# qwerty35/swarm_simulator

Hardware: AMD Instinct MI355X
Metric: agent-trajectories/sec (RBP plan: SFC+RSFC+QP) (higher is better)
Workload: dtype f64

## Files before the change

swarm_simulator_amd/csrc/abi/session.hip:

```cpp
#include <cmath>
#include <cstdio>
#include <cstdlib>
#include <cstring>
#include <string>
#include <thread>
#include <vector>

#include "../kernels/jqp.h"
#include "../kernels/rbp_dev.h"

namespace {

thread_local std::string g_err;

int fail(int code, const std::string& msg) {
    g_err = msg;
    return code;
}

#define HIP_TRY(expr)                                                                                    \
    do {                                                                                                 \
        hipError_t e_ = (expr);                                                                          \
        if (e_ != hipSuccess)                                                                            \
            return fail(e_ == hipErrorNoDevice || e_ == hipErrorInvalidDevice ? RBP_ERR_NO_DEVICE : RBP_ERR_HIP, \
// ... 490 lines not shown
    HIP_TRY(hipMemsetAsync(d.status, 0, sizeof(int) * K, st));
    HIP_TRY(hipMemsetAsync(d.scalars, 0, sizeof(double) * K * SC_N, st));
    HIP_TRY(hipMemsetAsync(d.counters, 0, sizeof(unsigned long long) * K * CT_N, st));
    if (s->have_corridor_inputs) {
        HIP_TRY(hipMemcpyAsync(d.sfc_count, s->sfc_count0.data(), sizeof(int) * (size_t)K * N, hipMemcpyHostToDevice, st));
        HIP_TRY(hipMemcpyAsync(d.sfc_box, s->sfc_box0.data(), sizeof(double) * (size_t)K * N * MB * 6, hipMemcpyHostToDevice, st));
        HIP_TRY(hipMemcpyAsync(d.sfc_time, s->sfc_time0.data(), sizeof(double) * (size_t)K * N * MB, hipMemcpyHostToDevice, st));
        HIP_TRY(hipMemcpyAsync(d.rsfc_normal, s->rsfc_normal0.data(), sizeof(float) * (size_t)K * d.npair * M * 3, hipMemcpyHostToDevice, st));
        HIP_TRY(hipMemcpyAsync(d.rsfc_time, s->rsfc_time0.data(), sizeof(double) * (size_t)K * M, hipMemcpyHostToDevice, st));
    }
    return RBP_OK;
}

int rbp_session_set_agent_range(rbp_session* s, int32_t agent_begin, int32_t agent_end) {
    if (!s) return fail(RBP_ERR_BAD_ARGUMENT, "null session");
    if (int jrc = join_worker(s)) return jrc;
    if (agent_begin < 0 || agent_end < agent_begin || agent_end > s->d.N) return fail(RBP_ERR_BAD_ARGUMENT, "agent range outside [0, N]");
    s->d.agent_begin = agent_begin, s->d.agent_end = agent_end;
    return RBP_OK;
}

static int ensure_planner_workspace(rbp_session* s, hipStream_t st) {
    const DevSession& d = s->d;
    const int N = d.N, M = d.M, K = d.K;
    const rbp_solver_opts& o = s->opts;
    const bool joint_wide = !s->param.sequential && s->biter > 0 && N >= 2 && o.joint_wide_min_agents > 0 && N >= o.joint_wide_min_agents;
    if (!joint_wide) {
        if (M > QP_MAX_M) return fail(RBP_ERR_BAD_ARGUMENT, "more than " + std::to_string(QP_MAX_M) + " segments per mission are not supported by the QP kernel");
        if (s->biter > 0 && s->bs > planner_max_batch())
            return fail(RBP_ERR_BAD_ARGUMENT, "batch wider than " + std::to_string(planner_max_batch()) +
                                                  " agents (joint QP of a large mission) is not supported by the one-workgroup QP kernel "
                                                  "(rbp_solver_opts.joint_wide_min_agents selects the grid-wide solver)");
    }
    const size_t per = joint_wide ? joint_workspace_bytes(N, M) : std::max(planner_workspace_bytes_w2(N, M, s->bs), planner_workspace_bytes_w4(N, M, s->bs));
    s->joint_wide = joint_wide;
    if (s->qp_ws && s->ws_joint == joint_wide && s->qp_ws_per_mission == per) return RBP_OK;
    const size_t total = per * (size_t)K + 256;
    auto too_large = [&](hipError_t e) {
        return fail(RBP_ERR_HIP, "QP workspace: " + std::to_string(total) + " bytes (" + std::to_string(K) + " missions x " + std::to_string(per) +
                                     " bytes for " + (joint_wide ? "the grid-wide joint solver" : "the batch QP kernels") + ") could not be reserved: " +
                                     hipGetErrorString(e));
    };
    char* base = nullptr;
    if (s->ctx) {
        rbp_ctx* c = s->ctx;
        if (c->ws_cap < total) {
            HIP_TRY(hipStreamSynchronize(st));
            if (c->ws_base) (void)hipFree(c->ws_base);
            c->ws_base = nullptr, c->ws_cap = 0;
            const size_t want = total + total / 4;
            hipError_t e = hipMalloc((void**)&c->ws_base, want);
            if (e != hipSuccess) return too_large(e);
            c->ws_cap = want;
        }
        base = c->ws_base;
    } else {
        if (s->ws_own) {
            HIP_TRY(hipStreamSynchronize(st));
            (void)hipFree(s->ws_own);
            s->ws_own = nullptr;
        }
        hipError_t e = hipMalloc((void**)&s->ws_own, total);
        if (e != hipSuccess) return too_large(e);
        base = s->ws_own;
    }
    HIP_TRY(hipMemsetAsync(base, 0, total, st));
    s->qp_ws = base, s->qp_ws_per_mission = per, s->ws_joint = joint_wide;
    return RBP_OK;
}

size_t rbp_session_workspace_bytes(rbp_session* s) { return s && s->qp_ws ? s->qp_ws_per_mission : 0; }

int rbp_session_reserve_workspace(rbp_session* s, void* stream) {
    if (!s) return fail(RBP_ERR_BAD_ARGUMENT, "null session");
    if (int jrc = join_worker(s)) return jrc;
    HIP_TRY(hipSetDevice(s->device));
    return ensure_planner_workspace(s, (hipStream_t)stream);
}

int rbp_session_set_solver_opts(rbp_session* s, const rbp_solver_opts* o) {
    if (!s) return fail(RBP_ERR_BAD_ARGUMENT, "null session");
    if (int jrc = join_worker(s)) return jrc;
    int rc = check_solver_opts(o);
    if (rc) return rc;
    s->opts = *o;
    return RBP_OK;
}

static int run_impl(rbp_session* s, int stages, void* stream, bool async) {
    if (!s) return fail(RBP_ERR_BAD_ARGUMENT, "null session");
    if (int jrc = join_worker(s)) return jrc;
    hipStream_t st = (hipStream_t)stream;
    HIP_TRY(hipSetDevice(s->device));
    const rbp_solver_opts& o = s->opts;
    if (stages & RBP_STAGE_PLANNER) {
        int rc = ensure_planner_workspace(s, st);
        if (rc) return rc;
        if (s->shard.nranks == 2 && !s->joint_wide)
            return fail(RBP_ERR_BAD_ARGUMENT, "rbp_session_shard_joint: this plan does not run on the grid-wide joint solver (rbp_solver_opts.joint_wide_min_agents), there is no factorisation to share");
        if (s->shard.nranks == 2 && async)
// ... 508 lines not shown
```

swarm_simulator_amd/csrc/kernels/qp.hip:

```cpp
#include <algorithm>
#include <type_traits>
#include <vector>

#include "rbp_dev.h"

#pragma clang fp contract(fast)

#include "knot_lds.inc"
#include "common/ipm_rows.h"

#ifndef QP_THREADS
#define QP_THREADS 512
#endif
#define QP_MAX_ITERS 80
#ifndef QP_WARM_TAU
#define QP_WARM_TAU 1e-3
#endif
#ifndef QP_MU0
#define QP_MU0 3e-1
#endif
#ifndef QP_ROW_UNROLL
#define QP_ROW_UNROLL 2
#endif
#ifndef QP_ROW_PF
// ... 8 lines not shown
#ifndef QP_FAR_SLACK
#define QP_FAR_SLACK 0.7
#endif
#ifndef QP_SIGMA_POW
#define QP_SIGMA_POW 3
#endif
#ifndef QP_NBHD_GAMMA
#define QP_NBHD_GAMMA 1e-3
#endif
#ifndef QP_NBHD_BACKOFF
#define QP_NBHD_BACKOFF 0.8
#endif
#ifndef QP_STEP_FRAC
#define QP_STEP_FRAC 0.997
#endif
#ifndef QP_SFLOOR
#define QP_SFLOOR 1e-1
#endif
#ifndef QP_WAVES_PER_EU
#define QP_WAVES_PER_EU 2
#endif
#ifndef QP_CHAIN_PRIO
#define QP_CHAIN_PRIO 3
#endif
#ifndef QP_STAGE_BUFS
#define QP_STAGE_BUFS (QP_THREADS >= 512 ? 3 : 2)
#endif
#ifndef QP_STAGE_REGS
#define QP_STAGE_REGS (QP_THREADS >= 512 ? 0 : 2)
#endif
#ifndef QP_MID_FOLLOW
#define QP_MID_FOLLOW (QP_THREADS >= 512)
#endif
#ifndef QP_FWD_IN_FACTOR
#ifdef QP_TRACE
#define QP_FWD_IN_FACTOR 0
#else
#define QP_FWD_IN_FACTOR 1
#endif
#endif
#if QP_FWD_IN_FACTOR && KL_FUSED_UPDATE && KL_PANEL && KL_PANEL_MIN_NK <= 36
#define QP_FWD36 1
#else
#define QP_FWD36 0
#endif
#ifndef QP_EARLY_TRIES
#define QP_EARLY_TRIES 2
#endif
#ifndef QP_EARLY_TOL
#define QP_EARLY_TOL 1e-6
#endif
#include "lh_layout.h"
#define PL_NC 256
#define PL_PMAX 160
#define PL_PBIG 192
__host__ __device__ inline int polish_pmax(int nk) { return nk <= 36 ? 112 : PL_PMAX; }
__host__ __device__ inline size_t polish_s_doubles(int nj) { return std::max((size_t)PL_NC * PL_NC, ipm::k0g_doubles(nj)); }
__host__ __device__ inline size_t polish_ws_doubles(int nj, int nk) {
    return 18 * (size_t)nj + 2 + ipm::k0g_doubles(nj) + PL_NC * 14 + polish_s_doubles(nj) + 8 + lhp_size(PL_PBIG) + 4 * 6 * PL_PBIG + 3 * (size_t)nj * nk;
}
__host__ __device__ inline int polish_lds_doubles(int nk) {
    const int pm = polish_pmax(nk);
    return lhp_size(pm) + 3 * PL_NC + 3 * pm + (pm + 2 * PL_NC + 8) / 2 + 8;
}

namespace {
using namespace ipm;

#include "qp_base.inc"
#include "qp_polish_types.inc"
#include "qp_rows.inc"
#include "qp_newton.inc"
#include "qp_wave_factor.inc"
#include "qp_wave_solve.inc"
#include "qp_tiled.inc"
#include "qp_entries.inc"
#include "qp_polish.inc"
#include "qp_batch.inc"

__global__ __launch_bounds__(QP_THREADS, QP_WAVES_PER_EU) void qp_batch_kernel(DevSession S, double* ws_base, size_t ws_stride, int passes,
                                                               int biter, int nbmax, int lds_doubles) {
    const int mission = S.qp_order ? __builtin_amdgcn_readfirstlane(S.qp_order[blockIdx.x]) : (int)blockIdx.x;
    const long long t_start = wall_clock64();
    __shared__ DevSession S_lds;
    if (threadIdx.x == 0) S_lds = S;
// ... 84 lines not shown
```

swarm_simulator_amd/csrc/kernels/qp_base.inc:

```

#ifdef QP_PROFILE
#define PROF_DECL long long prof_t0 = wall_clock64(), prof_acc[12] = {0, 0, 0, 0, 0, 0, 0, 0, 0, 0, 0, 0}
#define PROF(i)                                \
    do {                                       \
        __syncthreads();                       \
        long long t_ = wall_clock64();         \
        prof_acc[i] += t_ - prof_t0;           \
        prof_t0 = t_;                          \
    } while (0)
#define PROF_FLUSH(scal)                                                         \
    do {                                                                         \
        if (threadIdx.x == 0)                                                    \
            for (int i_ = 0; i_ < 12; ++i_) scal[SC_PROF0 + i_] += (double)prof_acc[i_]; \
    } while (0)
#else
#define PROF_DECL
#define PROF(i)
#define PROF_FLUSH(scal)
#endif

struct QpDims {
    int N, M, oq;
    int nb, NF, npb;
    int nk, nj, ld;
// ... 44 lines not shown
}

__host__ __device__ inline size_t ws_doubles(int N, int M, int nbmax) {
    QpDims d = make_dims(N, M, 0, nbmax);
    size_t n = 7 * d.nslot_max + 12 * (size_t)nbmax * d.oq + (size_t)(d.npb ? d.npb : 1) * d.oq + 3 * (size_t)nbmax * 3 * d.oq +
               2 * (size_t)d.nj * d.nk + (size_t)d.nj * d.ldb * d.ldb + 2 * (size_t)d.nj * (d.nk < 36 ? d.nk : 36) * (d.nk < 36 ? d.nk : 36) +
               (size_t)(d.nj > 1 ? d.nj - 1 : 1) * d.ldb * d.ldb + 4 +
               2 * (size_t)nbmax * M * 3 + 3 * (size_t)(M + 1) * 9 + M + 64 + (ws_int_count(N, M, nbmax) + 1) / 2 + 2 +
                polish_ws_doubles(d.nj, d.nk);
    return n;
}

__device__ inline QpWs carve(double* base, const QpDims& d, int nbmax) {
    QpDims dm = make_dims(d.N, d.M, 0, nbmax);
    QpWs w;
    double* p = base;
    w.s = p, p += dm.nslot_max;
    w.z = p, p += dm.nslot_max;
    w.s2 = p, p += dm.nslot_max;
    w.z2 = p, p += dm.nslot_max;
    w.rh = p, p += dm.nslot_max;
    w.cc = p, p += dm.nslot_max;
    w.ds = p, p += dm.nslot_max;
    w.cpacc = p, p += 12 * (size_t)nbmax * d.oq;
    w.pwgt = p, p += (size_t)(dm.npb ? dm.npb : 1) * d.oq;
    w.dx = p, p += (size_t)nbmax * 3 * d.oq;
    w.dxa = p, p += (size_t)nbmax * 3 * d.oq;
    w.cvec = p, p += (size_t)nbmax * 3 * d.oq;
    w.rbase = p, p += (size_t)dm.nj * dm.nk;
    w.rhs = p, p += (size_t)dm.nj * dm.nk;
    p += (4 - ((p - base) & 3)) & 3;
    w.Td = p, p += (size_t)dm.nj * dm.ldb * dm.ldb;
    w.To = p, p += (size_t)(dm.nj > 1 ? dm.nj - 1 : 1) * dm.ldb * dm.ldb;
    w.Lf = p, p += 2 * (size_t)dm.nj * (dm.nk < 36 ? dm.nk : 36) * (dm.nk < 36 ? dm.nk : 36);
    w.boxlo = p, p += (size_t)nbmax * d.M * 3;
    w.boxhi = p, p += (size_t)nbmax * d.M * 3;
    w.Lk = p, p += (size_t)(d.M + 1) * 9;
    w.Dk = p, p += (size_t)(d.M + 1) * 9;
    w.Ek = p, p += (size_t)(d.M + 1) * 9;
    w.segsc = p, p += d.M;
    int* ip = (int*)p;
    w.flist = ip, ip += (size_t)nbmax * d.M * d.N;
    w.fnear = ip, ip += (size_t)nbmax * d.M;
    w.fcnt = ip, ip += (size_t)nbmax * d.M;
    w.fbase = ip, ip += (size_t)nbmax * d.M;
    w.fperm = ip, ip += (size_t)nbmax * d.M;
    w.frank = ip, ip += (size_t)nbmax * d.M;
    w.tile_base = ip, ip += dm.ntile + 1;
    w.wi_of = ip, ip += (size_t)nbmax * d.oq;
    w.nrm = (float*)ip;
    w.polish = p + (ws_int_count(d.N, d.M, nbmax) + 1) / 2 + 2;
    w.prof = nullptr;
    return w;
}

template <int CTRL>
__device__ __forceinline__ double dpp_f64(double v) {
    const int lo = __builtin_amdgcn_update_dpp(0, __double2loint(v), CTRL, 0xf, 0xf, false);
    const int hi = __builtin_amdgcn_update_dpp(0, __double2hiint(v), CTRL, 0xf, 0xf, false);
    return __hiloint2double(hi, lo);
}
__device__ __forceinline__ double red_op(double a, double b, int op) { return op == 0 ? a + b : (op == 1 ? fmax(a, b) : fmin(a, b)); }
__device__ __forceinline__ double rl(double v, int lane) {
    return __hiloint2double(__builtin_amdgcn_readlane(__double2hiint(v), lane), __builtin_amdgcn_readlane(__double2loint(v), lane));
}
__device__ __forceinline__ double wave_red(double v, int op ) {
    v = red_op(v, dpp_f64<0xB1>(v), op);
// ... 103 lines not shown
```

swarm_simulator_amd/csrc/kernels/qp_batch.inc:

```

#ifdef QP_TRACE
#ifndef QP_TRACE_BATCH
#define QP_TRACE_BATCH 0
#endif
#define TRC(slot, expr)                                                         \
    do {                                                                        \
        if (batch == QP_TRACE_BATCH && pass_index == 0 && iter < 100) {                       \
            const double v_ = (expr);                                           \
            if (tid == 0) trc[iter * 16 + (slot)] = v_;                         \
        }                                                                       \
    } while (0)
__device__ double trc_sum(const double* p, size_t n, double* red) {
    double a = 0;
    for (size_t i = threadIdx.x; i < n; i += QP_THREADS) a += fabs(p[i]);
    return block_reduce(a, 0, red);
}
#else
#define TRC(slot, expr)
#endif

__device__ __forceinline__ bool qp_setup_batch(const DevSession& S, RowCtx& c, double* ctrl, const double* T, int mission, int first, int nb,
                                               int* flag, double* lds, int& frozen_free_rows, double far_R, int& nfar) {
    const int tid = threadIdx.x, N = S.N;
    const QpDims& d = c.d;
// ... 326 lines not shown
        const bool early = early_tries < QP_EARLY_TRIES && pres < QP_EARLY_TOL && dres < QP_EARLY_TOL &&
                           mu < (early_tries == 0 ? QP_EARLY_TOL : 1e-2 * QP_EARLY_TOL);
        if (S.p.polish && (polish_first || early)) {
            if (!polish_first) early_tries++;
            const int acc = polish_entry(c, pw, lds, red, flag, polish_first ? 1 : 0);
            __syncthreads();
            PROF(0);
#ifdef QP_POLSTATS
            if (tid == 0 && !polish_first) scal[25] += (early_tries == 1), scal[26] += (early_tries == 1 && acc == 0), scal[27] += (early_tries == 2), scal[29] += (early_tries == 2 && acc == 0);
#endif
            if (acc == 0) {
                ok = true, polished = 1;
                break;
            }
        }
        if (d.nk > 36)
            assemble_blocks(c, lds);
        else if (ASM_HELPERS == 0 && !QP_FOLLOW_ASM)
            assemble_blocks_lds(asm_args(c), d.nj, lds);
#if QP_FWD36
        if (d.nk == 36) rhs_from_acc(c, false, 0.0);
#endif
        PROF(3);
        __threadfence_block();
        __syncthreads();
        TRC(5, trc_sum(w.Td, (size_t)d.nj * d.ldb * d.ldb, red));
        if (!factor_entry(ba, asm_args(c), lds, flag)) {
            fail_reason = 2;
            break;
        }
        flops += d.nk <= 36 ? (double)d.nj * ((7.0 / 6.0) * d.nk * (double)d.nk * d.nk + 6.0 * d.nk * (double)d.nk)
                            : (double)d.nj * (7.0 / 3.0) * d.nk * (double)d.nk * d.nk;
        PROF(4);
        TRC(6, trc_sum(d.nk <= 36 ? w.Lf : w.Td, d.nk <= 36 ? (size_t)d.nj * 2 * d.nk * d.nk : (size_t)d.nj * d.ldb * d.ldb, red));
#ifndef QP_TRACE
        if (d.nk <= 36) {
            PROF(5);
            #if QP_FWD36
            solve_entry(ba, w.rhs, lds, SolveOut{w.dxa, w.Lk, d.oq, d.nk == 36 ? 3 : 1, w.cpacc, w.rbase, 0.0});
#else
            solve_entry(ba, w.rhs, lds, SolveOut{w.dxa, w.Lk, d.oq, 1, w.cpacc, w.rbase, 0.0});
#endif
            PROF(6);
        } else
#endif
        {
            rhs_from_acc(c, false, 0.0);
            __threadfence_block();
            __syncthreads();
            PROF(5);
            TRC(7, trc_sum(w.rhs, (size_t)d.nj * d.nk, red));
            solve_entry(ba, w.rhs, lds);
            PROF(6);
            TRC(8, trc_sum(w.rhs, (size_t)d.nj * d.nk, red));
            apply_F(d, w, w.rhs, w.dxa);
            __threadfence_block();
            __syncthreads();
        }
        io.sum0 = io.sum1 = io.sum2 = 0, io.vmax = 1.0;
        PROF(5);
        SWEEP(PASS_AFF);
        PROF(7);
        const double a_aff = 1.0 / block_reduce(io.vmax, 1, red);
        const double q0 = block_reduce(io.sum0, 0, red), q1 = block_reduce(io.sum1, 0, red), q2 = block_reduce(io.sum2, 0, red);
        const double mu_aff = (q0 + a_aff * q1 + a_aff * a_aff * q2) / nrows_free;
        TRC(9, a_aff); TRC(10, mu_aff);
        double sigma = mu_aff / mu;
// ... 203 lines not shown
```

swarm_simulator_amd/csrc/kernels/qp_wave_factor.inc:

```

__device__ __forceinline__ int twist_mid(int nj) { return nj / 2; }

#define ASM_WAVE0 4
#define ASM_HELPERS (QP_THREADS / 64 > ASM_WAVE0 ? QP_THREADS / 64 - ASM_WAVE0 : 0)
#ifndef QP_FOLLOW_ASM
#define QP_FOLLOW_ASM (ASM_HELPERS == 0)
#endif
#define ASMF_READY(cnt, h) ((kl_ldsi*)((cnt) + 76 + (h)))
__device__ __forceinline__ void wait_blocks(int* cnt, int i) {
    while (__hip_atomic_load(cnt + i, __ATOMIC_RELAXED, __HIP_MEMORY_SCOPE_WORKGROUP) < ASM_HELPERS) __builtin_amdgcn_s_sleep(2);
    __builtin_amdgcn_fence(__ATOMIC_ACQUIRE, "workgroup");
}

typedef double d4 __attribute__((ext_vector_type(4)));

template <int NK>
__device__ __forceinline__ bool chol_rows(double (&a)[NK], double& dinv) {
    bool ok = true;
    const int r = threadIdx.x & 63;
    dinv = 1.0;
#pragma unroll
    for (int c = 0; c < NK; ++c) {
        const double dcc = rl(a[c], c);
        if (!(dcc > 0)) ok = false;
        const double inv = fast_rsqrt(dcc);
        dinv = (r == c) ? inv : dinv;
        a[c] *= inv;
#pragma unroll
        for (int k = c + 1; k < NK; ++k) a[k] -= a[c] * rl(a[c], k);
    }
    return ok;
}

#define KF_STRIDE(NK) ((NK) * (NK) + KL_I)

__device__ __forceinline__ void coupling_coef(const QpWs& w, int j, int dir, int rr, double& e0, double& e1, double& e2) {
    const __attribute__((address_space(1))) double* E = QGC(w.Ek) + 9 * (dir > 0 ? j + 1 : j);
    e0 = dir > 0 ? E[rr % 3] : E[3 * (rr % 3)], e1 = dir > 0 ? E[3 + rr % 3] : E[3 * (rr % 3) + 1],
    e2 = dir > 0 ? E[6 + rr % 3] : E[3 * (rr % 3) + 2];
}

template <int NK>
__device__ __forceinline__ bool knot_ldl(const QpWs& w, int j, bool minus_u, kl_lds* base, int r, bool act, int rr, kl_ldsi* P, int pbase,
                                         const kl_lds* Timg = nullptr, kl_ldsi* consumed = nullptr, int consumed_value = 0) {
    using A = KlArea<NK>;
    kl_lds *C = base + A::C, *I = base + A::I, *U = base + A::C;
    if constexpr (kl_panel_path(NK)) {
        if (Timg)
            return kl_knot_panels<NK, true>([&](int mx, int mn) { return (double)Timg[mn * KL_LD + mx]; },
                                      [&] {
                                          kl_sync();
                                          if (consumed) kl_publish(consumed, consumed_value);
                                      },
                                      minus_u, C, I, r, P, pbase);
        const double* Tg = w.Td + (size_t)j * NK * NK;
        return kl_knot_panels<NK, false>([&](int mx, int mn) { return Tg[mn * NK + mx]; }, [] {}, minus_u, C, I, r, P, pbase);
    }
    double a[NK];
    if (Timg) {
#pragma unroll
        for (int k = 0; k < NK; ++k) a[k] = Timg[k * KL_LD + rr];
        kl_sync();
        if (consumed) kl_publish(consumed, consumed_value);
    } else {
        const double* Tg = w.Td + (size_t)j * NK * NK;
#pragma unroll
        for (int k = 0; k < NK; ++k) a[k] = Tg[k * NK + rr];
// ... 4 lines not shown
        kl_sync();
    }
    return kl_ldl<NK>(a, C, I, r, act, P, pbase);
}

template <int NK>
__device__ __forceinline__ bool knot_ldl_add(const QpWs& w, int j, kl_d4 (&s)[KlPanels<NK>::TILES], kl_lds* base, int r, kl_ldsi* P, int pbase,
                                             const kl_lds* Timg = nullptr, kl_ldsi* consumed = nullptr, int consumed_value = 0) {
    using A = KlArea<NK>;
    kl_lds *C = base + A::C, *I = base + A::I;
    if (Timg)
        return kl_knot_panels_add<NK, true>(s, [&](int mx, int mn) { return (double)Timg[mn * KL_LD + mx]; },
                                            [&] {
                                                kl_sync();
                                                if (consumed) kl_publish(consumed, consumed_value);
                                            },
                                            C, I, r, P, pbase);
    const double* Tg = w.Td + (size_t)j * NK * NK;
    return kl_knot_panels_add<NK, false>(s, [&](int mx, int mn) { return Tg[mn * NK + mx]; }, [] {}, C, I, r, P, pbase);
}
template <int NK>
__device__ __forceinline__ void fused_coupling_coef(const QpWs& w, int j, int dir, int lane, double (&cf)[KlPanels<NK>::NT][3]) {
    const __attribute__((address_space(1))) double* E = QGC(w.Ek) + 9 * (dir > 0 ? j + 1 : j);
    kl_fused_coef<NK>(cf, lane, [&](int row, int q) { return dir > 0 ? E[3 * q + row % 3] : E[3 * (row % 3) + q]; });
}

template <int NK, bool FOLLOW>
__device__ __forceinline__ void knot_inverse(const QpWs& w, int j, kl_lds* base, int r, bool act, kl_ldsi* P, int pbase, int& seen, kl_ldsi* Mdone,
                                             int done_value) {
    using A = KlArea<NK>;
    kl_lds *C = base + A::C, *MX = base + A::MX, *I = base + A::I;
    double m[NK];
    const double dinv = kl_inverse_rows<NK, FOLLOW>(m, C, I, MX, r, act, P, pbase, Mdone, done_value);
    __attribute__((address_space(1))) double* Mg = QG(w.Lf + (size_t)j * KF_STRIDE(NK));
    if (FOLLOW && QP_FOLLOW_ASM) asm volatile("s_waitcnt vmcnt(0)" ::: "memory");
    if (act) {
        __attribute__((address_space(1))) double* row = Mg + (size_t)r * NK;
        if ((NK & 1) == 0) {
#pragma unroll
            for (int k = 0; k < NK; k += 2)
                if (k + 1 >= r) *(__attribute__((address_space(1))) kl_d2*)(row + k) = kl_d2{m[k], m[k + 1]};
        } else {
#pragma unroll
            for (int k = 0; k < NK; ++k)
                if (k >= r) row[k] = m[k];
        }
        Mg[NK * NK + r] = dinv;
    }
}

#if defined(QP_PROFILE) && !defined(QP_LHSTATS) && !defined(QP_SOLVE_TIMERS)
#define CHAIN_TW(cnt, slot) ((__attribute__((address_space(3))) unsigned long long*)((cnt) + 96) + ((slot) - 25))
#define CHAIN_T0 long long ct_ = wall_clock64()
#define CHAIN_T(slot)                                                                                                                              \
    do {                                                                                                                                           \
        const long long t_ = wall_clock64();                                                                                                       \
        __hip_atomic_fetch_add(CHAIN_TW(cnt, slot), (dir > 0 && r == 0) ? (unsigned long long)(t_ - ct_) : 0ull, __ATOMIC_RELAXED, __HIP_MEMORY_SCOPE_WORKGROUP); \
        ct_ = t_;                                                                                                                                  \
    } while (0)
#define CHAIN_FLUSH()                                                                                   \
    do {                                                                                                \
        kl_sync();                                                                                      \
        if (w.prof && dir > 0 && r == 0)                                                                \
            for (int k_ = 25; k_ < 28; ++k_) w.prof[k_] += (double)(long long)*CHAIN_TW(cnt, k_);       \
        if (QP_FWD_IN_FACTOR && w.prof && dir > 0 && r == 0) w.prof[29] += (double)(long long)*CHAIN_TW(cnt, 29); \
    } while (0)
#else
#define CHAIN_T0
#define CHAIN_T(slot)
#define CHAIN_FLUSH()
#endif
#define CHAIN_SYNC(cnt, h) ((kl_ldsi*)((cnt) + 64 + 2 * (h)))
#define ASM_CONSUMED(cnt, h) ((kl_ldsi*)((cnt) + 72 + (h)))

static_assert((QP_FWD36 != 0) == (QP_FWD_IN_FACTOR && kl_fused_path(36)), "QP_FWD36 (qp.hip) out of step with kl_fused_path");
template <int NK>
__device__ __forceinline__ void wave_forward_step(const QpWs& w, kl_lds* base, int jp, double rhs_r, double e0, double e1, double e2, int r) {
    kl_forward_step<NK>(base, QG(w.rhs) + (size_t)jp * NK + (r < NK ? r : 0), rhs_r, e0, e1, e2, r);
}
template <int NK>
// ... 250 lines not shown
```

swarm_simulator_amd/csrc/kernels/qp_wave_solve.inc:

```

#include "knot_subst.h"

template <int NK>
struct KsLayout {
    static constexpr int SM = NK * KL_LD, SCH = SM + KL_I, STG = 2 * SCH;
    static constexpr int LEAD = 16;
    static constexpr int VECS = 6 * KS_VLEN + 2 * 64;
};

struct SolveOut {
    double* dx_out;
    const double* Lk;
    int oq;
    int rhs_mode = 0;
    const double* cpacc = nullptr;
    const double* rbase = nullptr;
    double sigma_mu = 0;
};
template <int NK, int ROLE>
__device__ __forceinline__ void solve_staged(const QpDims& d, const QpWs& w, double* rhs, double* lds, SolveOut so = SolveOut{nullptr, nullptr, 0}) {
    using KS = KsLayout<NK>;
    constexpr int STG = KS::STG, SCH = KS::SCH, SM = KS::SM;
    const int tid = threadIdx.x, nj = d.nj, mid = twist_mid(nj);
    const int nl = mid, nr = nj - 1 - mid, SF = nl > nr ? nl : nr;
    const int nsteps = 2 * SF + 1;
    constexpr bool FWD = QP_FWD_IN_FACTOR && kl_fused_path(NK);
    const bool bwd_only = FWD && so.rhs_mode == 3;
    const int s_first = bwd_only ? SF + 1 : 0;
    lds += KS::LEAD;
    kl_lds* vec = (kl_lds*)(lds + QP_STAGE_BUFS * STG);
    kl_lds* small = vec + ((nj * NK + 1) & ~1);
    if (FWD ? so.rhs_mode == 1 || so.rhs_mode == 2 : so.rhs_mode != 0) {
        constexpr int nu = NK / 3;
        const int oq = so.oq;
        const size_t ncp = (size_t)(NK / 9) * oq;
        const bool corrector = so.rhs_mode == 2;
        for (int it = tid; it < nj * nu; it += QP_THREADS) {
            const int j = it / nu + 1, u = it % nu, a = u / 3, k = u % 3;
            double g[6];
#pragma unroll
            for (int q = 0; q < 6; ++q) {
                const int j6 = 6 * (j - 1) + 3 + q;
                const __attribute__((address_space(1))) double* ac = QGC(so.cpacc) + (size_t)a * oq + j6;
                g[q] = corrector ? ac[k * ncp] - so.sigma_mu * ac[(3 + k) * ncp] : ac[(6 + k) * ncp];
            }
            const __attribute__((address_space(1))) double* L = QGC(so.Lk) + 9 * j;
            const size_t o0 = (size_t)(j - 1) * NK + u * 3;
#pragma unroll
            for (int e = 0; e < 3; ++e) vec[o0 + e] = QGC(so.rbase)[o0 + e] + g[3 + e] + L[0 + e] * g[0] + L[3 + e] * g[1] + L[6 + e] * g[2];
        }
    } else {
        constexpr int RQ = 4;
        for (int i0 = tid; i0 < nj * NK; i0 += RQ * QP_THREADS) {
            double t[RQ];
#pragma unroll
            for (int q = 0; q < RQ; ++q) t[q] = i0 + q * QP_THREADS < nj * NK ? rhs[i0 + q * QP_THREADS] : 0.0;
#pragma unroll
            for (int q = 0; q < RQ; ++q)
                if (i0 + q * QP_THREADS < nj * NK) vec[i0 + q * QP_THREADS] = t[q];
        }
    }
    for (int i = tid; i < KS::VECS; i += QP_THREADS) small[i] = 0.0;
    auto left_j = [&](int s) { return s < SF ? (s - (SF - nl) >= 0 ? s - (SF - nl) : -1) : (s == SF ? mid : (mid - 1 - (s - SF - 1) >= 0 ? mid - 1 - (s - SF - 1) : -1)); };
    auto right_j = [&](int s) { return s < SF ? (s - (SF - nr) >= 0 ? nj - 1 - (s - (SF - nr)) : -1) : (s == SF ? -1 : (mid + 1 + (s - SF - 1) <= nj - 1 ? mid + 1 + (s - SF - 1) : -1)); };
    constexpr int NTRI = NK * (NK + 1) / 2, NE = NTRI + NK, NST = QP_THREADS - 128, MAXE = (2 * NE + NST - 1) / NST;
    int soff[MAXE], doff[MAXE];
    if (ROLE == 1) {
#pragma unroll
        for (int u = 0; u < MAXE; ++u) {
            const int e = (tid - 128) + u * NST;
            soff[u] = 0, doff[u] = -1;
            if (e < 2 * NE) {
                const int side = e >= NE, idx = side ? e - NE : e;
                if (idx < NTRI) {
                    int rw = (int)(((2 * NK + 1) - sqrtf((float)((2 * NK + 1) * (2 * NK + 1) - 8 * idx))) * 0.5f);
                    if (rw * NK - rw * (rw - 1) / 2 > idx) rw--;
                    if ((rw + 1) * NK - (rw + 1) * rw / 2 <= idx) rw++;
                    const int k = rw + idx - (rw * NK - rw * (rw - 1) / 2);
                    soff[u] = rw * NK + k, doff[u] = side * SCH + rw * KL_LD + k;
                } else {
                    soff[u] = NK * NK + (idx - NTRI), doff[u] = side * SCH + SM + (idx - NTRI);
                }
            }
        }
    }
    for (int i = tid; i < KS::LEAD + QP_STAGE_BUFS * STG; i += QP_THREADS) (lds - KS::LEAD)[i] = 0.0;
    __syncthreads();
    if (bwd_only && tid < NK) small[KS_VPAD + 2 * KS_VLEN + tid] = small[KS_VPAD + 5 * KS_VLEN + tid] = vec[mid * NK + tid];
    auto stage = [&](int s, double* buf) {
        const int jl = left_j(s), jr = right_j(s);
        const double* srcl = w.Lf + (size_t)(jl >= 0 ? jl : 0) * KF_STRIDE(NK);
        const double* srcr = w.Lf + (size_t)(jr >= 0 ? jr : 0) * KF_STRIDE(NK);
        double tmp[MAXE];
#pragma unroll
        for (int u = 0; u < MAXE; ++u) {
            const bool right = doff[u] >= SCH;
            const bool on = doff[u] >= 0 && (right ? jr >= 0 : jl >= 0);
            tmp[u] = on ? (right ? srcr : srcl)[soff[u]] : 0.0;
        }
#pragma unroll
        for (int u = 0; u < MAXE; ++u) {
            const bool right = doff[u] >= SCH;
            if (doff[u] >= 0 && (right ? jr >= 0 : jl >= 0)) buf[doff[u]] = tmp[u];
        }
    };
    auto stage_load = [&](int s, double (&tmp)[MAXE]) {
        if (s >= nsteps) return;
        const int jl = left_j(s), jr = right_j(s);
        typedef __attribute__((address_space(1))) const double gdbl;
        gdbl* srcl = (gdbl*)(w.Lf + (size_t)(jl >= 0 ? jl : 0) * KF_STRIDE(NK));
        gdbl* srcr = (gdbl*)(w.Lf + (size_t)(jr >= 0 ? jr : 0) * KF_STRIDE(NK));
#pragma unroll
        for (int u = 0; u < MAXE; ++u) tmp[u] = (doff[u] >= SCH ? srcr : srcl)[soff[u]];
    };
    auto stage_store = [&](int s, const double (&tmp)[MAXE], double* buf) {
        if (s >= nsteps) return;
        const int jl = left_j(s), jr = right_j(s);
        kl_lds* bl = (kl_lds*)buf;
#pragma unroll
        for (int u = 0; u < MAXE; ++u) {
            const bool right = doff[u] >= SCH;
            if (doff[u] >= 0 && (right ? jr >= 0 : jl >= 0)) bl[doff[u]] = tmp[u];
        }
    };
    if (ROLE == 1)
        for (int s0 = s_first; s0 < s_first + QP_STAGE_BUFS - 1 && s0 < nsteps; ++s0) stage(s0, lds + (bwd_only ? s0 % QP_STAGE_BUFS : s0) * STG);
    __syncthreads();
    const int wave = ROLE == 0 ? (tid >> 6) & 1 : 2, r = tid & 63;
    const bool act = r < NK;
    const int rr = act ? r : 0, g3 = 3 * (rr / 3), r3 = rr % 3;
    const int rs = act ? r : NK + 12;
    if (wave < 2) __builtin_amdgcn_s_setprio(QP_CHAIN_PRIO);
    auto step_coef = [&](int s, double& q0, double& q1, double& q2) {
        q0 = q1 = q2 = 0.0;
        if (ROLE != 0 || s >= nsteps || s == SF) return;
        const int jb = wave == 0 ? left_j(s) : right_j(s);
        if (jb < 0) return;
        const int dir = wave == 0 ? +1 : -1;
        if (s < SF) {
            const bool has_prev = wave == 0 ? jb > 0 : jb + 1 < nj;
            if (has_prev) coupling_coef(w, jb - dir, dir, rr, q0, q1, q2);
        } else {
            const __attribute__((address_space(1))) double* E = QGC(w.Ek) + 9 * (dir > 0 ? jb + 1 : jb);
            q0 = dir > 0 ? E[3 * r3] : E[r3], q1 = dir > 0 ? E[3 * r3 + 1] : E[3 + r3], q2 = dir > 0 ? E[3 * r3 + 2] : E[6 + r3];
        }
    };
    double cf0, cf1, cf2;
    step_coef(s_first, cf0, cf1, cf2);
#ifdef QP_SOLVE_TIMERS
    long long st_ = wall_clock64();
#define SOLVE_T(slot)                                                              \
    do {                                                                           \
        const long long t_ = wall_clock64();                                       \
        const int who_ = ROLE == 0 ? (tid == 0 ? 0 : (tid == 64 ? 8 : -1)) : (tid == 128 ? 4 : -1);  \
        if (w.prof && who_ >= 0) w.prof[slot + who_] += (double)(t_ - st_);        \
        st_ = t_;                                                                  \
    } while (0)
#else
#define SOLVE_T(slot)
#endif
    if (ROLE == 1 && QP_STAGE_REGS > 0) {
        constexpr int R = QP_STAGE_REGS > 0 ? QP_STAGE_REGS : 1;
        double tq[R][MAXE];
#pragma unroll
        for (int k = 0; k < R; ++k) stage_load(s_first + QP_STAGE_BUFS - 1 + k, tq[k]);
        int dsto[MAXE];
#pragma unroll
        for (int u = 0; u < MAXE; ++u) dsto[u] = doff[u] >= 0 ? doff[u] : KL_LD - 1;
        typedef __attribute__((address_space(1))) const double gdbl;
        double nq[R][MAXE];
        int s = s_first;
        for (; s + 2 * R + QP_STAGE_BUFS - 1 <= nsteps; s += R) {
#pragma unroll
            for (int k = 0; k < R; ++k) {
                const int sl = s + R + k + QP_STAGE_BUFS - 1;
                const int jl = left_j(sl), jr = right_j(sl);
                gdbl* srcl = (gdbl*)(w.Lf + (size_t)(jl >= 0 ? jl : 0) * KF_STRIDE(NK));
                gdbl* srcr = (gdbl*)(w.Lf + (size_t)(jr >= 0 ? jr : 0) * KF_STRIDE(NK));
#pragma unroll
                for (int u = 0; u < MAXE; ++u) nq[k][u] = (doff[u] >= SCH ? srcr : srcl)[soff[u]];
            }
#pragma unroll
            for (int k = 0; k < R; ++k) {
                const int sp = s + k + QP_STAGE_BUFS - 1;
                kl_lds* bl = (kl_lds*)(lds + (sp % QP_STAGE_BUFS) * STG);
#pragma unroll
                for (int u = 0; u < MAXE; ++u) bl[dsto[u]] = tq[k][u];
                __syncthreads();
            }
#pragma unroll
            for (int k = 0; k < R; ++k)
#pragma unroll
                for (int u = 0; u < MAXE; ++u) tq[k][u] = nq[k][u];
        }
        for (; s < nsteps; s += R) {
#pragma unroll
            for (int k = 0; k < R; ++k) {
                if (s + k < nsteps) {
                    const int sp = s + k + QP_STAGE_BUFS - 1;
                    stage_store(sp, tq[k], lds + (sp % QP_STAGE_BUFS) * STG);
                    stage_load(sp + R, tq[k]);
                    __syncthreads();
                }
            }
        }
    } else
    for (int s = s_first; s < nsteps; ++s) {
        SOLVE_T(26);
        const double e0 = cf0, e1 = cf1, e2 = cf2;
        step_coef(s + 1, cf0, cf1, cf2);
        double* buf = lds + (s % QP_STAGE_BUFS) * STG;
        if (ROLE == 1) {
            const int sp = s + QP_STAGE_BUFS - 1;
            if (sp < nsteps) stage(sp, lds + (sp % QP_STAGE_BUFS) * STG);
        } else if (s == SF) {
            if (wave == 0) {
                const kl_lds* Mst = (const kl_lds*)buf;
                kl_lds *A0 = (kl_lds*)small + KS_VPAD, *Z0 = A0 + KS_VLEN, *V0 = A0 + 2 * KS_VLEN, *V1 = A0 + 5 * KS_VLEN;
                kl_lds* ps = (kl_lds*)small + 6 * KS_VLEN;
                double v = vec[mid * NK + rr];
// ... 62 lines not shown
```

Baseline: 194,700.

## Pack knot factor rows into an upper-triangular layout with 16-byte staging loads

Stores each knot's inverse-factor block in a packed upper-triangular layout (row pairs for even NK) instead of a full NK×NK square, and stages it into LDS as 16-byte units, so fewer and wider global loads are issued per solve step. Workspace and the Lf region are aligned to 128/16-byte boundaries to make the vector loads legal. The packed path is enabled only when QP_THREADS < 512; the default 512-thread build keeps the square layout and mainly gets the alignment plus the lambda reorganisation. Index math for packed offsets adds some setup cost.

```diff
diff --git a/swarm_simulator_amd/csrc/abi/session.hip b/swarm_simulator_amd/csrc/abi/session.hip
--- a/swarm_simulator_amd/csrc/abi/session.hip
+++ b/swarm_simulator_amd/csrc/abi/session.hip
@@ -546,7 +546,8 @@
                                                   " agents (joint QP of a large mission) is not supported by the one-workgroup QP kernel "
                                                   "(rbp_solver_opts.joint_wide_min_agents selects the grid-wide solver)");
     }
-    const size_t per = joint_wide ? joint_workspace_bytes(N, M) : std::max(planner_workspace_bytes_w2(N, M, s->bs), planner_workspace_bytes_w4(N, M, s->bs));
+    const size_t per = joint_wide ? joint_workspace_bytes(N, M)
+                                  : (std::max(planner_workspace_bytes_w2(N, M, s->bs), planner_workspace_bytes_w4(N, M, s->bs)) + 127) & ~size_t(127);
     s->joint_wide = joint_wide;
     if (s->qp_ws && s->ws_joint == joint_wide && s->qp_ws_per_mission == per) return RBP_OK;
     const size_t total = per * (size_t)K + 256;
@@ -579,7 +580,7 @@
         base = s->ws_own;
     }
     HIP_TRY(hipMemsetAsync(base, 0, total, st));
-    s->qp_ws = base, s->qp_ws_per_mission = per, s->ws_joint = joint_wide;
+    s->qp_ws = base + (128 - (size_t)base % 128) % 128, s->qp_ws_per_mission = per, s->ws_joint = joint_wide;
     return RBP_OK;
 }
 
diff --git a/swarm_simulator_amd/csrc/kernels/knot_factor_layout.h b/swarm_simulator_amd/csrc/kernels/knot_factor_layout.h
--- /dev/null
+++ b/swarm_simulator_amd/csrc/kernels/knot_factor_layout.h
@@ -0,0 +1,44 @@
+#pragma once
+#ifndef KF_FN
+#define KF_FN __host__ __device__ inline
+#endif
+
+KF_FN constexpr int kf_first(int nk, int r) { return (nk & 1) ? r : (r & ~1); }
+KF_FN constexpr int kf_len(int nk, int r) { return nk - kf_first(nk, r); }
+KF_FN constexpr int kf_row(int nk, int r) {
+    return (nk & 1) ? r * nk - r * (r - 1) / 2 : 2 * (r / 2) * nk - 2 * (r / 2) * (r / 2 - 1) + (r & 1) * (nk - (r & ~1));
+}
+KF_FN constexpr int kf_elem(int nk, int r, int k) { return kf_row(nk, r) + k - kf_first(nk, r); }
+KF_FN constexpr int kf_tri(int nk) { return kf_row(nk, nk); }
+KF_FN constexpr int kf_dinv(int nk) { return (kf_tri(nk) + 1) & ~1; }
+KF_FN constexpr int kf_run(int nk) { return kf_dinv(nk) + nk; }
+KF_FN constexpr int kf_stride(int nk) { return (kf_run(nk) + 15) & ~15; }
+
+KF_FN constexpr int kf_sq_elem(int nk, int r, int k) { return r * nk + k; }
+KF_FN constexpr int kf_sq_dinv(int nk) { return nk * nk; }
+KF_FN constexpr int kf_sq_stride(int nk) { return nk * nk + 40; }
+
+KF_FN constexpr int kf_unit(int nk) { return (nk & 1) ? 1 : 2;  }
+KF_FN constexpr int kf_units(int nk) { return (kf_run(nk) + kf_unit(nk) - 1) / kf_unit(nk); }
+KF_FN constexpr int kf_unit_side(int nk, int e) { return e >= kf_units(nk) ? 1 : 0; }
+KF_FN constexpr int kf_unit_off(int nk, int e) { return (e - kf_unit_side(nk, e) * kf_units(nk)) * kf_unit(nk); }
+KF_FN int kf_row_of(int nk, int o) {
+    int r;
+    if (nk & 1) {
+        const float b = (float)(2 * nk + 1);
+        r = (int)((b - __builtin_sqrtf(b * b - 8.0f * (float)o)) * 0.5f);
+    } else {
+        const float b = (float)(nk + 1);
+        r = 2 * (int)((b - __builtin_sqrtf(b * b - 2.0f * (float)o)) * 0.5f);
+    }
+    r = r < 0 ? 0 : (r > nk - 1 ? nk - 1 : r);
+    while (r > 0 && kf_row(nk, r) > o) --r;
+    while (r + 1 < nk && kf_row(nk, r + 1) <= o) ++r;
+    return r;
+}
+KF_FN int kf_stage_dst(int nk, int o, int ld, int sm) {
+    if (o >= kf_dinv(nk)) return o < kf_run(nk) ? sm + (o - kf_dinv(nk)) : -1;
+    if (o >= kf_tri(nk)) return -1;
+    const int r = kf_row_of(nk, o);
+    return r * ld + kf_first(nk, r) + (o - kf_row(nk, r));
+}
diff --git a/swarm_simulator_amd/csrc/kernels/qp.hip b/swarm_simulator_amd/csrc/kernels/qp.hip
--- a/swarm_simulator_amd/csrc/kernels/qp.hip
+++ b/swarm_simulator_amd/csrc/kernels/qp.hip
@@ -64,6 +64,9 @@
 #ifndef QP_MID_FOLLOW
 #define QP_MID_FOLLOW (QP_THREADS >= 512)
 #endif
+#ifndef QP_LF_PACKED
+#define QP_LF_PACKED (QP_THREADS >= 512 ? 0 : 1)
+#endif
 #ifndef QP_FWD_IN_FACTOR
 #ifdef QP_TRACE
 #define QP_FWD_IN_FACTOR 0
@@ -83,6 +86,7 @@
 #define QP_EARLY_TOL 1e-6
 #endif
 #include "lh_layout.h"
+#include "knot_factor_layout.h"
 #define PL_NC 256
 #define PL_PMAX 160
 #define PL_PBIG 192
diff --git a/swarm_simulator_amd/csrc/kernels/qp_base.inc b/swarm_simulator_amd/csrc/kernels/qp_base.inc
--- a/swarm_simulator_amd/csrc/kernels/qp_base.inc
+++ b/swarm_simulator_amd/csrc/kernels/qp_base.inc
@@ -100,7 +100,7 @@
     p += (4 - ((p - base) & 3)) & 3;
     w.Td = p, p += (size_t)dm.nj * dm.ldb * dm.ldb;
     w.To = p, p += (size_t)(dm.nj > 1 ? dm.nj - 1 : 1) * dm.ldb * dm.ldb;
-    w.Lf = p, p += 2 * (size_t)dm.nj * (dm.nk < 36 ? dm.nk : 36) * (dm.nk < 36 ? dm.nk : 36);
+    w.Lf = p + ((16 - ((p - base) & 15)) & 15), p += 2 * (size_t)dm.nj * (dm.nk < 36 ? dm.nk : 36) * (dm.nk < 36 ? dm.nk : 36);
     w.boxlo = p, p += (size_t)nbmax * d.M * 3;
     w.boxhi = p, p += (size_t)nbmax * d.M * 3;
     w.Lk = p, p += (size_t)(d.M + 1) * 9;
diff --git a/swarm_simulator_amd/csrc/kernels/qp_batch.inc b/swarm_simulator_amd/csrc/kernels/qp_batch.inc
--- a/swarm_simulator_amd/csrc/kernels/qp_batch.inc
+++ b/swarm_simulator_amd/csrc/kernels/qp_batch.inc
@@ -382,7 +382,7 @@
         flops += d.nk <= 36 ? (double)d.nj * ((7.0 / 6.0) * d.nk * (double)d.nk * d.nk + 6.0 * d.nk * (double)d.nk)
                             : (double)d.nj * (7.0 / 3.0) * d.nk * (double)d.nk * d.nk;
         PROF(4);
-        TRC(6, trc_sum(d.nk <= 36 ? w.Lf : w.Td, d.nk <= 36 ? (size_t)d.nj * 2 * d.nk * d.nk : (size_t)d.nj * d.ldb * d.ldb, red));
+        TRC(6, trc_sum(d.nk <= 36 ? w.Lf : w.Td, d.nk <= 36 ? (size_t)d.nj * (QP_LF_PACKED ? kf_stride(d.nk) : kf_sq_stride(d.nk)) : (size_t)d.nj * d.ldb * d.ldb, red));
 #ifndef QP_TRACE
         if (d.nk <= 36) {
             PROF(5);
diff --git a/swarm_simulator_amd/csrc/kernels/qp_wave_factor.inc b/swarm_simulator_amd/csrc/kernels/qp_wave_factor.inc
--- a/swarm_simulator_amd/csrc/kernels/qp_wave_factor.inc
+++ b/swarm_simulator_amd/csrc/kernels/qp_wave_factor.inc
@@ -32,7 +32,18 @@
     return ok;
 }
 
-#define KF_STRIDE(NK) ((NK) * (NK) + KL_I)
+#if QP_LF_PACKED
+#define KF_SLOT(NK) kf_stride(NK)
+#define KF_ELEM(NK, r, k) kf_elem(NK, r, k)
+#define KF_DINV(NK) kf_dinv(NK)
+#else
+static_assert(KL_I == 40, "kf_sq_stride (knot_factor_layout.h) restates KL_I");
+#define KF_SLOT(NK) kf_sq_stride(NK)
+#define KF_ELEM(NK, r, k) kf_sq_elem(NK, r, k)
+#define KF_DINV(NK) kf_sq_dinv(NK)
+#endif
+static_assert(KF_SLOT(9) + 15 <= 2 * 81 && KF_SLOT(18) + 15 <= 2 * 324 && KF_SLOT(27) + 15 <= 2 * 729 && KF_SLOT(36) + 15 <= 2 * 1296,
+              "a knot's slot and the doubles in front of the first one fit the region carve() gives QpWs::Lf");
 
 __device__ __forceinline__ void coupling_coef(const QpWs& w, int j, int dir, int rr, double& e0, double& e1, double& e2) {
     const __attribute__((address_space(1))) double* E = QGC(w.Ek) + 9 * (dir > 0 ? j + 1 : j);
@@ -103,10 +114,10 @@
     kl_lds *C = base + A::C, *MX = base + A::MX, *I = base + A::I;
     double m[NK];
     const double dinv = kl_inverse_rows<NK, FOLLOW>(m, C, I, MX, r, act, P, pbase, Mdone, done_value);
-    __attribute__((address_space(1))) double* Mg = QG(w.Lf + (size_t)j * KF_STRIDE(NK));
+    __attribute__((address_space(1))) double* Mg = QG(w.Lf + (size_t)j * KF_SLOT(NK));
     if (FOLLOW && QP_FOLLOW_ASM) asm volatile("s_waitcnt vmcnt(0)" ::: "memory");
     if (act) {
-        __attribute__((address_space(1))) double* row = Mg + (size_t)r * NK;
+        __attribute__((address_space(1))) double* row = Mg + KF_ELEM(NK, r, 0);
         if ((NK & 1) == 0) {
 #pragma unroll
             for (int k = 0; k < NK; k += 2)
@@ -116,7 +127,7 @@
             for (int k = 0; k < NK; ++k)
                 if (k >= r) row[k] = m[k];
         }
-        Mg[NK * NK + r] = dinv;
+        Mg[KF_DINV(NK) + r] = dinv;
     }
 }
 
diff --git a/swarm_simulator_amd/csrc/kernels/qp_wave_solve.inc b/swarm_simulator_amd/csrc/kernels/qp_wave_solve.inc
--- a/swarm_simulator_amd/csrc/kernels/qp_wave_solve.inc
+++ b/swarm_simulator_amd/csrc/kernels/qp_wave_solve.inc
@@ -30,6 +30,73 @@
     lds += KS::LEAD;
     kl_lds* vec = (kl_lds*)(lds + QP_STAGE_BUFS * STG);
     kl_lds* small = vec + ((nj * NK + 1) & ~1);
+    auto left_j = [&](int s) { return s < SF ? (s - (SF - nl) >= 0 ? s - (SF - nl) : -1) : (s == SF ? mid : (mid - 1 - (s - SF - 1) >= 0 ? mid - 1 - (s - SF - 1) : -1)); };
+    auto right_j = [&](int s) { return s < SF ? (s - (SF - nr) >= 0 ? nj - 1 - (s - (SF - nr)) : -1) : (s == SF ? -1 : (mid + 1 + (s - SF - 1) <= nj - 1 ? mid + 1 + (s - SF - 1) : -1)); };
+    constexpr bool PK = QP_LF_PACKED != 0;
+    constexpr int NTRI = NK * (NK + 1) / 2, NE = NTRI + NK;
+    constexpr int UN = PK ? kf_unit(NK) : 1, NU = PK ? kf_units(NK) : NE;
+    constexpr int NST = QP_THREADS - 128, MAXE = (2 * NU + NST - 1) / NST;
+    typedef typename std::conditional<UN == 2, kl_d2, double>::type unit_t;
+    typedef __attribute__((address_space(1))) const double gdbl;
+    typedef __attribute__((address_space(1))) const unit_t gunit;
+    typedef __attribute__((address_space(3))) unit_t lunit;
+    static_assert(UN == 1 || (KL_LD % 2 == 0 && SM % 2 == 0 && SCH % 2 == 0 && STG % 2 == 0 && KS::LEAD % 2 == 0), "16-byte units: even offsets in a stage");
+    int doff[MAXE];
+    [[maybe_unused]] int soff[PK ? 1 : MAXE];
+    if (ROLE == 1) {
+#pragma unroll
+        for (int u = 0; u < MAXE; ++u) {
+            const int e = (tid - 128) + u * NST;
+            doff[u] = -1;
+            if constexpr (!PK) soff[u] = 0;
+            if (e < 2 * NU) {
+                [[maybe_unused]] const int side = e >= NU, idx = side ? e - NU : e;
+                if constexpr (PK) {
+                    const int dd = kf_stage_dst(NK, kf_unit_off(NK, e), KL_LD, SM);
+                    doff[u] = dd >= 0 ? kf_unit_side(NK, e) * SCH + dd : -1;
+                } else if (idx < NTRI) {
+                    int rw = (int)(((2 * NK + 1) - sqrtf((float)((2 * NK + 1) * (2 * NK + 1) - 8 * idx))) * 0.5f);
+                    if (rw * NK - rw * (rw - 1) / 2 > idx) rw--;
+                    if ((rw + 1) * NK - (rw + 1) * rw / 2 <= idx) rw++;
+                    const int k = rw + idx - (rw * NK - rw * (rw - 1) / 2);
+                    soff[u] = KF_ELEM(NK, rw, k), doff[u] = side * SCH + rw * KL_LD + k;
+                } else {
+                    soff[u] = KF_DINV(NK) + (idx - NTRI), doff[u] = side * SCH + SM + (idx - NTRI);
+                }
+            }
+        }
+    }
+    auto unit_src = [&](int u, gdbl* srcl, gdbl* srcr) {
+        if constexpr (PK) {
+            const int e = (tid - 128) + u * NST;
+            return (gunit*)((kf_unit_side(NK, e) ? srcr : srcl) + (e < 2 * NU ? kf_unit_off(NK, e) : 0));
+        } else {
+            return (gunit*)((doff[u] >= SCH ? srcr : srcl) + soff[u]);
+        }
+    };
+    auto stage_load = [&](int s, unit_t (&tmp)[MAXE]) {
+        if (s >= nsteps) return;
+        const int jl = left_j(s), jr = right_j(s);
+        gdbl* srcl = (gdbl*)(w.Lf + (size_t)(jl >= 0 ? jl : 0) * KF_SLOT(NK));
+        gdbl* srcr = (gdbl*)(w.Lf + (size_t)(jr >= 0 ? jr : 0) * KF_SLOT(NK));
+#pragma unroll
+        for (int u = 0; u < MAXE; ++u) tmp[u] = *unit_src(u, srcl, srcr);
+    };
+    auto stage_store = [&](int s, const unit_t (&tmp)[MAXE], double* buf) {
+        if (s >= nsteps) return;
+        const int jl = left_j(s), jr = right_j(s);
+        kl_lds* bl = (kl_lds*)buf;
+#pragma unroll
+        for (int u = 0; u < MAXE; ++u) {
+            const bool right = doff[u] >= SCH;
+            if (doff[u] >= 0 && (right ? jr >= 0 : jl >= 0)) *(lunit*)(bl + doff[u]) = tmp[u];
+        }
+    };
+    auto stage = [&](int s, double* buf) {
+        unit_t tmp[MAXE];
+        stage_load(s, tmp);
+        stage_store(s, tmp, buf);
+    };
     if (FWD ? so.rhs_mode == 1 || so.rhs_mode == 2 : so.rhs_mode != 0) {
         constexpr int nu = NK / 3;
         const int oq = so.oq;
@@ -61,70 +128,11 @@
         }
     }
     for (int i = tid; i < KS::VECS; i += QP_THREADS) small[i] = 0.0;
-    auto left_j = [&](int s) { return s < SF ? (s - (SF - nl) >= 0 ? s - (SF - nl) : -1) : (s == SF ? mid : (mid - 1 - (s - SF - 1) >= 0 ? mid - 1 - (s - SF - 1) : -1)); };
-    auto right_j = [&](int s) { return s < SF ? (s - (SF - nr) >= 0 ? nj - 1 - (s - (SF - nr)) : -1) : (s == SF ? -1 : (mid + 1 + (s - SF - 1) <= nj - 1 ? mid + 1 + (s - SF - 1) : -1)); };
-    constexpr int NTRI = NK * (NK + 1) / 2, NE = NTRI + NK, NST = QP_THREADS - 128, MAXE = (2 * NE + NST - 1) / NST;
-    int soff[MAXE], doff[MAXE];
-    if (ROLE == 1) {
-#pragma unroll
-        for (int u = 0; u < MAXE; ++u) {
-            const int e = (tid - 128) + u * NST;
-            soff[u] = 0, doff[u] = -1;
-            if (e < 2 * NE) {
-                const int side = e >= NE, idx = side ? e - NE : e;
-                if (idx < NTRI) {
-                    int rw = (int)(((2 * NK + 1) - sqrtf((float)((2 * NK + 1) * (2 * NK + 1) - 8 * idx))) * 0.5f);
-                    if (rw * NK - rw * (rw - 1) / 2 > idx) rw--;
-                    if ((rw + 1) * NK - (rw + 1) * rw / 2 <= idx) rw++;
-                    const int k = rw + idx - (rw * NK - rw * (rw - 1) / 2);
-                    soff[u] = rw * NK + k, doff[u] = side * SCH + rw * KL_LD + k;
-                } else {
-                    soff[u] = NK * NK + (idx - NTRI), doff[u] = side * SCH + SM + (idx - NTRI);
-                }
-            }
-        }
-    }
     for (int i = tid; i < KS::LEAD + QP_STAGE_BUFS * STG; i += QP_THREADS) (lds - KS::LEAD)[i] = 0.0;
     __syncthreads();
     if (bwd_only && tid < NK) small[KS_VPAD + 2 * KS_VLEN + tid] = small[KS_VPAD + 5 * KS_VLEN + tid] = vec[mid * NK + tid];
-    auto stage = [&](int s, double* buf) {
-        const int jl = left_j(s), jr = right_j(s);
-        const double* srcl = w.Lf + (size_t)(jl >= 0 ? jl : 0) * KF_STRIDE(NK);
-        const double* srcr = w.Lf + (size_t)(jr >= 0 ? jr : 0) * KF_STRIDE(NK);
-        double tmp[MAXE];
-#pragma unroll
-        for (int u = 0; u < MAXE; ++u) {
-            const bool right = doff[u] >= SCH;
-            const bool on = doff[u] >= 0 && (right ? jr >= 0 : jl >= 0);
-            tmp[u] = on ? (right ? srcr : srcl)[soff[u]] : 0.0;
-        }
-#pragma unroll
-        for (int u = 0; u < MAXE; ++u) {
-            const bool right = doff[u] >= SCH;
-            if (doff[u] >= 0 && (right ? jr >= 0 : jl >= 0)) buf[doff[u]] = tmp[u];
-        }
-    };
-    auto stage_load = [&](int s, double (&tmp)[MAXE]) {
-        if (s >= nsteps) return;
-        const int jl = left_j(s), jr = right_j(s);
-        typedef __attribute__((address_space(1))) const double gdbl;
-        gdbl* srcl = (gdbl*)(w.Lf + (size_t)(jl >= 0 ? jl : 0) * KF_STRIDE(NK));
-        gdbl* srcr = (gdbl*)(w.Lf + (size_t)(jr >= 0 ? jr : 0) * KF_STRIDE(NK));
-#pragma unroll
-        for (int u = 0; u < MAXE; ++u) tmp[u] = (doff[u] >= SCH ? srcr : srcl)[soff[u]];
-    };
-    auto stage_store = [&](int s, const double (&tmp)[MAXE], double* buf) {
-        if (s >= nsteps) return;
-        const int jl = left_j(s), jr = right_j(s);
-        kl_lds* bl = (kl_lds*)buf;
-#pragma unroll
-        for (int u = 0; u < MAXE; ++u) {
-            const bool right = doff[u] >= SCH;
-            if (doff[u] >= 0 && (right ? jr >= 0 : jl >= 0)) bl[doff[u]] = tmp[u];
-        }
-    };
     if (ROLE == 1)
-        for (int s0 = s_first; s0 < s_first + QP_STAGE_BUFS - 1 && s0 < nsteps; ++s0) stage(s0, lds + (bwd_only ? s0 % QP_STAGE_BUFS : s0) * STG);
+        for (int s0 = s_first; s0 < s_first + QP_STAGE_BUFS - 1 && s0 < nsteps; ++s0) stage(s0, lds + (s0 % QP_STAGE_BUFS) * STG);
     __syncthreads();
     const int wave = ROLE == 0 ? (tid >> 6) & 1 : 2, r = tid & 63;
     const bool act = r < NK;
@@ -161,31 +169,32 @@
 #endif
     if (ROLE == 1 && QP_STAGE_REGS > 0) {
         constexpr int R = QP_STAGE_REGS > 0 ? QP_STAGE_REGS : 1;
-        double tq[R][MAXE];
+        unit_t tq[R][MAXE];
 #pragma unroll
         for (int k = 0; k < R; ++k) stage_load(s_first + QP_STAGE_BUFS - 1 + k, tq[k]);
+        constexpr int DUMP = UN == 2 ? NK : KL_LD - 1;
+        static_assert(DUMP + UN <= KL_LD, "the padding columns of row 0");
         int dsto[MAXE];
 #pragma unroll
-        for (int u = 0; u < MAXE; ++u) dsto[u] = doff[u] >= 0 ? doff[u] : KL_LD - 1;
-        typedef __attribute__((address_space(1))) const double gdbl;
-        double nq[R][MAXE];
+        for (int u = 0; u < MAXE; ++u) dsto[u] = doff[u] >= 0 ? doff[u] : DUMP;
+        unit_t nq[R][MAXE];
         int s = s_first;
         for (; s + 2 * R + QP_STAGE_BUFS - 1 <= nsteps; s += R) {
 #pragma unroll
             for (int k = 0; k < R; ++k) {
                 const int sl = s + R + k + QP_STAGE_BUFS - 1;
                 const int jl = left_j(sl), jr = right_j(sl);
-                gdbl* srcl = (gdbl*)(w.Lf + (size_t)(jl >= 0 ? jl : 0) * KF_STRIDE(NK));
-                gdbl* srcr = (gdbl*)(w.Lf + (size_t)(jr >= 0 ? jr : 0) * KF_STRIDE(NK));
-#pragma unroll
-                for (int u = 0; u < MAXE; ++u) nq[k][u] = (doff[u] >= SCH ? srcr : srcl)[soff[u]];
+                gdbl* srcl = (gdbl*)(w.Lf + (size_t)(jl >= 0 ? jl : 0) * KF_SLOT(NK));
+                gdbl* srcr = (gdbl*)(w.Lf + (size_t)(jr >= 0 ? jr : 0) * KF_SLOT(NK));
+#pragma unroll
+                for (int u = 0; u < MAXE; ++u) nq[k][u] = *unit_src(u, srcl, srcr);
             }
 #pragma unroll
             for (int k = 0; k < R; ++k) {
                 const int sp = s + k + QP_STAGE_BUFS - 1;
                 kl_lds* bl = (kl_lds*)(lds + (sp % QP_STAGE_BUFS) * STG);
 #pragma unroll
-                for (int u = 0; u < MAXE; ++u) bl[dsto[u]] = tq[k][u];
+                for (int u = 0; u < MAXE; ++u) *(lunit*)(bl + dsto[u]) = tq[k][u];
                 __syncthreads();
             }
 #pragma unroll
```

Measured after the change: 199,500 (median of 6 runs). +2.4%, better.
